# zafarrafii/REPET-Python

Hardware: AMD Instinct MI355X
Metric: audio-seconds/sec (x real-time) for repet.sim, 44.1 kHz stereo (higher is better)
Workload: dtype f32 (similarity GEMM: f16x3 split of the fp32 unit rows, fp32 accumulate; median: exact selection on bit-sliced rank codes)

## Files before the change

### repet-python_amd/csrc/peaks_exact.hip

```cpp
#include "peaks.h"
#include "fft_wave_f64.h"

#include <algorithm>
#include <cstdlib>
#include <type_traits>

namespace repet {

namespace {

#ifdef REPET_EXACT_STAMPS
#define XSTAMP_DECL unsigned long long xlast_ = wall_clock64();
#define XSTAMP(k) { __syncthreads(); if (threadIdx.x == 0) { const unsigned long long now_ = wall_clock64(); atomicAdd(&stats[24 + (k)], (unsigned)(now_ - xlast_)); xlast_ = now_; } }
#else
#define XSTAMP_DECL
#define XSTAMP(k)
#endif

#ifdef REPET_EXACT_STAMPS
__device__ unsigned long long g_unit_stamps[8];
#define USTAMP(k) { const unsigned long long now_ = wall_clock64(); if (lane == 0) atomicAdd(&g_unit_stamps[k], now_ - ulast_); ulast_ = now_; }
#define USTAMP_DECL unsigned long long ulast_ = wall_clock64();
#else
#define USTAMP(k)
#define USTAMP_DECL
#endif
constexpr int kExactThreads = 256, kExactWaves = kExactThreads / 64;
constexpr int kScanChunk = 4096;
constexpr int kRankLds = 512;
constexpr unsigned int kNear = 1, kSure = 2, kNeed1 = 4, kNeed2 = 8, kBand = 128;

struct ExactArgs {
    PeakArgs a;
    double delta2;
    const int* redo_list;
    ExactSource src;
    unsigned gen;
    int logM;
    unsigned char* scratch; size_t scratch_per_wg; int n4;
    int tw_count, fft_waves, wave_bytes, scan_in_lds;
    int reg_fft;
};

struct RowScratch {
    float* v; double* val; unsigned long long* best; unsigned int* st; int* list; int* list2; int* near; float* pval; int* pidx; int* prank;
};

__host__ __device__ inline size_t exact_row_scratch_bytes(int n4) {
    return (size_t)n4 * (8 + 8 + 4 + 4 + 4 + 4 + 4 + 4 + 4 + 4) + 256;
}

__device__ __forceinline__ RowScratch carve_row(unsigned char* p, int n4) {
    RowScratch r;
    r.val = reinterpret_cast<double*>(p); p += (size_t)n4 * 8;
    r.best = reinterpret_cast<unsigned long long*>(p); p += (size_t)n4 * 8;
    r.v = reinterpret_cast<float*>(p); p += (size_t)n4 * 4;
    r.list = reinterpret_cast<int*>(p); p += (size_t)n4 * 4;
    r.near = reinterpret_cast<int*>(p); p += (size_t)n4 * 4;
    r.pval = reinterpret_cast<float*>(p); p += (size_t)n4 * 4;
    r.pidx = reinterpret_cast<int*>(p); p += (size_t)n4 * 4;
    r.prank = reinterpret_cast<int*>(p); p += (size_t)n4 * 4;
    r.list2 = reinterpret_cast<int*>(p); p += (size_t)n4 * 4;
    r.st = reinterpret_cast<unsigned int*>(p);
    return r;
}

__device__ __forceinline__ void exact_wave_sync() {
    __builtin_amdgcn_fence(__ATOMIC_RELEASE, "wavefront");
    __builtin_amdgcn_wave_barrier();
    __builtin_amdgcn_fence(__ATOMIC_ACQUIRE, "wavefront");
}

template <bool ACC_REGS, bool STOCKHAM>
__device__ __forceinline__ void wave_unit_row_f64(const ExactSource& s, int logM, int clip, int64_t fr, double2* Zw, double* accw, const double2* tws, int lane) {
    const int W = s.W, M = W >> 1, F = s.F, C = s.n_channels;
    const int64_t s0 = s.frame_sample0 + fr * (int64_t)s.H;
    const float* hi = s.hi + (int64_t)clip * s.clip_stride;
    const float* lo = s.lo ? s.lo + (int64_t)clip * s.clip_stride : nullptr;
    const float* lo_or_hi = lo ? lo : hi;
    const double lo_scale = lo ? 1.0 : 0.0;
    int rel_lo = (int)min(max(-s0, (int64_t)0), (int64_t)W);
    int rel_hi = (int)min(max(s.n_samples - s0, (int64_t)0), (int64_t)W);
    const bool none = rel_hi <= rel_lo;
    const int64_t anchor = none ? 0 : s0;
    if (none) rel_hi = rel_lo + 1;
    const float* frame_hi = hi + anchor * C;
    const float* frame_lo = lo_or_hi + anchor * C;
    constexpr int kAcc = ACC_REGS ? 17 : 1;
    double acc[kAcc];
#pragma unroll
    for (int jj = 0; jj < kAcc; ++jj) acc[jj] = 0.0;
    if (!ACC_REGS) for (int k = lane; k <= M; k += 64) accw[k] = 0.0;
    for (int c = 0; c < C; ++c) {
        exact_wave_sync();
        for (int r0 = 0; r0 < M; r0 += 512) {
            float h0[8], h1[8], l0[8], l1[8];
            double w0[8], w1[8];
#pragma unroll
            for (int u = 0; u < 8; ++u) {
                const int r = min(r0 + 64 * u + lane, M - 1);
                const int q0 = min(max(2 * r, rel_lo), rel_hi - 1), q1 = min(max(2 * r + 1, rel_lo), rel_hi - 1);
                h0[u] = frame_hi[q0 * C + c]; h1[u] = frame_hi[q1 * C + c];
                l0[u] = frame_lo[q0 * C + c]; l1[u] = frame_lo[q1 * C + c];
                w0[u] = s.window64[2 * r]; w1[u] = s.window64[2 * r + 1];
            }
#pragma unroll
            for (int u = 0; u < 8; ++u) {
                const int r = r0 + 64 * u + lane;
                const int p0 = 2 * r;
                const bool in0 = !none && p0 >= rel_lo && p0 < rel_hi, in1 = !none && p0 + 1 >= rel_lo && p0 + 1 < rel_hi;
                const double re = in0 ? ((double)h0[u] + lo_scale * (double)l0[u]) * w0[u] : 0.0;
                const double im = in1 ? ((double)h1[u] + lo_scale * (double)l1[u]) * w1[u] : 0.0;
                if (r < M) Zw[STOCKHAM ? r : (int)(__brev((unsigned)r) >> (32 - logM))] = make_double2(re, im);
            }
        }
        exact_wave_sync();
        if constexpr (STOCKHAM) {
            for (int p = 1; p < M;) {
                if (M / p >= 4) {
                    const int tstep = M / (p * 4);
                    double2 u[4][4];
#pragma unroll
                    for (int b = 0; b < 4; ++b) {
                        const int i = min(lane + 64 * b, (M >> 2) - 1);
                        u[b][0] = Zw[i]; u[b][1] = Zw[i + (M >> 2)]; u[b][2] = Zw[i + (M >> 1)]; u[b][3] = Zw[i + 3 * (M >> 2)];
                    }
                    exact_wave_sync();
#pragma unroll
                    for (int b = 0; b < 4; ++b) {
                        const int i = lane + 64 * b;
                        if (i < (M >> 2)) {
                            const int k = i & (p - 1);
                            const int j = ((i - k) << 2) + k;
                            double2 u0 = u[b][0], u1 = u[b][1], u2 = u[b][2], u3 = u[b][3];
                            if (p > 1) {
                                const double2 w1 = tws[k * tstep], w2 = tws[2 * k * tstep], w3 = tws[3 * k * tstep];
                                u1 = make_double2(u1.x * w1.x - u1.y * w1.y, u1.x * w1.y + u1.y * w1.x);
                                u2 = make_double2(u2.x * w2.x - u2.y * w2.y, u2.x * w2.y + u2.y * w2.x);
                                u3 = make_double2(u3.x * w3.x - u3.y * w3.y, u3.x * w3.y + u3.y * w3.x);
                            }
                            const double2 t0 = make_double2(u0.x + u2.x, u0.y + u2.y), t1 = make_double2(u0.x - u2.x, u0.y - u2.y);
                            const double2 t2 = make_double2(u1.x + u3.x, u1.y + u3.y), d = make_double2(u1.x - u3.x, u1.y - u3.y);
                            const double2 t3 = make_double2(d.y, -d.x);
                            Zw[j] = make_double2(t0.x + t2.x, t0.y + t2.y);
                            Zw[j + p] = make_double2(t1.x + t3.x, t1.y + t3.y);
                            Zw[j + 2 * p] = make_double2(t0.x - t2.x, t0.y - t2.y);
                            Zw[j + 3 * p] = make_double2(t1.x - t3.x, t1.y - t3.y);
                        }
                    }
                    p *= 4;
                } else {
                    const int tstep = M / (p * 2);
                    double2 u[8][2];
#pragma unroll
                    for (int b = 0; b < 8; ++b) {
                        const int i = min(lane + 64 * b, (M >> 1) - 1);
                        u[b][0] = Zw[i]; u[b][1] = Zw[i + (M >> 1)];
                    }
                    exact_wave_sync();
#pragma unroll
                    for (int b = 0; b < 8; ++b) {
                        const int i = lane + 64 * b;
                        if (i < (M >> 1)) {
                            const int k = i & (p - 1);
                            const int j = ((i - k) << 1) + k;
                            const double2 w1 = tws[k * tstep];
                            const double2 u1 = make_double2(u[b][1].x * w1.x - u[b][1].y * w1.y, u[b][1].x * w1.y + u[b][1].y * w1.x);
                            Zw[j] = make_double2(u[b][0].x + u1.x, u[b][0].y + u1.y);
                            Zw[j + p] = make_double2(u[b][0].x - u1.x, u[b][0].y - u1.y);
                        }
                    }
                    p *= 2;
                }
                exact_wave_sync();
            }
        } else {
        for (int h = 1; h < M; h <<= 1) {
                const int ts = M / (2 * h);
                for (int b = lane; b < (M >> 1); b += 64) {
                    const int k = b & (h - 1);
                    const int i0 = ((b - k) << 1) + k, i1 = i0 + h;
                    const double2 w = tws ? tws[k * ts] : s.twiddle64[2 * k * ts];
                    const double2 u = Zw[i0], t = Zw[i1];
                    const double tr = t.x * w.x - t.y * w.y, ti = t.x * w.y + t.y * w.x;
                    Zw[i0] = make_double2(u.x + tr, u.y + ti);
                    Zw[i1] = make_double2(u.x - tr, u.y - ti);
                }
                exact_wave_sync();
            }
        }
        auto magnitude = [&](int k, double2 w) -> double {
            const double2 a = Zw[k & (M - 1)], b = Zw[(M - k) & (M - 1)];
            const double er = 0.5 * (a.x + b.x), ei = 0.5 * (a.y - b.y);
            const double dr = 0.5 * (a.x - b.x), di = 0.5 * (a.y + b.y);
            const double orr = di, oi = -dr;
            const double xr = er + orr * w.x - oi * w.y, xi = ei + orr * w.y + oi * w.x;
            return sqrt(xr * xr + xi * xi);
        };
        if (ACC_REGS) {
            double2 w[kAcc];
#pragma unroll
            for (int jj = 0; jj < kAcc; ++jj) w[jj] = s.twiddle64[min(lane + 64 * jj, M)];
#pragma unroll
            for (int jj = 0; jj < kAcc; ++jj) { const int k = min(lane + 64 * jj, M); const double m = magnitude(k, w[jj]); acc[jj] += (lane + 64 * jj <= M) ? m : 0.0; }
        } else {
            for (int k0 = 0; k0 <= M; k0 += 512) {
                double2 w[8];
#pragma unroll
                for (int u = 0; u < 8; ++u) w[u] = s.twiddle64[min(k0 + 64 * u + lane, M)];
#pragma unroll
                for (int u = 0; u < 8; ++u) { const int k = k0 + 64 * u + lane; if (k <= M) accw[k] += magnitude(k, w[u]); }
            }
        }
    }
    double part = 0.0;
    if (ACC_REGS) {
#pragma unroll
        for (int jj = 0; jj < kAcc; ++jj) { const int k = lane + 64 * jj; acc[jj] = acc[jj] / (double)C; if (k < F) part += acc[jj] * acc[jj]; }
    } else {
        exact_wave_sync();
        for (int k = lane; k < F; k += 64) { const double m = accw[k] / (double)C; accw[k] = m; part += m * m; }
        exact_wave_sync();
    }
    const double nrm = sqrt(wave_sum_f64(part));
    const bool mute = s.silent_zero && nrm == 0.0;
    double* out = s.u64 + (int64_t)clip * s.u64_clip_stride + fr * (int64_t)s.FS;
    if (ACC_REGS) {
#pragma unroll
        for (int jj = 0; jj < kAcc; ++jj) { const int k = lane + 64 * jj; if (k < s.FS) out[k] = (k < F && !mute) ? acc[jj] / nrm : 0.0; }
    } else {
        for (int k = lane; k < s.FS; k += 64) out[k] = (k < F && !mute) ? accw[k] / nrm : 0.0;
    }
}

__device__ __forceinline__ void wave_unit_row_f64_reg(const ExactSource& s, int clip, int64_t fr, double2* ex, const f64fft::Twiddles& tw, int lane) {
    constexpr int M = f64fft::kRegN;
    const int F = s.F, C = s.n_channels;
    const int64_t s0 = s.frame_sample0 + fr * (int64_t)s.H;
    const float* hi = s.hi + (int64_t)clip * s.clip_stride;
    const float* lo = s.lo ? s.lo + (int64_t)clip * s.clip_stride : nullptr;
    const float* lo_or_hi = lo ? lo : hi;
    const double lo_scale = lo ? 1.0 : 0.0;
    const int W2 = 2 * M;
    int rel_lo = (int)min(max(-s0, (int64_t)0), (int64_t)W2);
    int rel_hi = (int)min(max(s.n_samples - s0, (int64_t)0), (int64_t)W2);
    const bool none = rel_hi <= rel_lo;
    const int64_t anchor = none ? 0 : s0;
    if (none) rel_hi = rel_lo + 1;
    const float* frame_hi = hi + anchor * C;
    const float* frame_lo = lo_or_hi + anchor * C;
    double acc[17];
#pragma unroll
    for (int jj = 0; jj < 17; ++jj) acc[jj] = 0.0;
    USTAMP_DECL
    for (int c = 0; c < C; ++c) {
        double2 v[16];
        const bool pair_ok = !none && rel_lo == 0 && rel_hi == W2;
        if (pair_ok && C == 2) {
            struct __attribute__((packed, aligned(4))) F4 { float x, y, z, w; };
#pragma unroll
            for (int half = 0; half < 2; ++half) {
                float4 h4[8], l4[8];
                double2 w[8];
#pragma unroll
                for (int u = 0; u < 8; ++u) {
                    const int r = 64 * (8 * half + u) + lane;
                    const F4 a4 = *reinterpret_cast<const F4*>(frame_hi + 4 * r), b4 = *reinterpret_cast<const F4*>(frame_lo + 4 * r);
                    h4[u] = make_float4(a4.x, a4.y, a4.z, a4.w); l4[u] = make_float4(b4.x, b4.y, b4.z, b4.w);
                    w[u] = *reinterpret_cast<const double2*>(s.window64 + 2 * r);
                }
#pragma unroll
                for (int u = 0; u < 8; ++u) {
                    const float a0 = c ? h4[u].y : h4[u].x, a1 = c ? h4[u].w : h4[u].z, b0 = c ? l4[u].y : l4[u].x, b1 = c ? l4[u].w : l4[u].z;
                    v[8 * half + u] = make_double2(((double)a0 + lo_scale * (double)b0) * w[u].x, ((double)a1 + lo_scale * (double)b1) * w[u].y);
                }
                __builtin_amdgcn_sched_barrier(0);
            }
        } else if (pair_ok && C == 1) {
            struct __attribute__((packed, aligned(4))) F2 { float x, y; };
#pragma unroll
            for (int u = 0; u < 16; ++u) {
                const int r = 64 * u + lane;
                const F2 a2 = *reinterpret_cast<const F2*>(frame_hi + 2 * r), b2 = *reinterpret_cast<const F2*>(frame_lo + 2 * r);
                const double2 w = *reinterpret_cast<const double2*>(s.window64 + 2 * r);
                v[u] = make_double2(((double)a2.x + lo_scale * (double)b2.x) * w.x, ((double)a2.y + lo_scale * (double)b2.y) * w.y);
            }
            __builtin_amdgcn_sched_barrier(0);
        } else {
#pragma unroll
        for (int half = 0; half < 2; ++half) {
            float h0[8], h1[8], l0[8], l1[8];
            double2 w[8];
#pragma unroll
            for (int u = 0; u < 8; ++u) {
                const int r = 64 * (8 * half + u) + lane;
                const int q0 = min(max(2 * r, rel_lo), rel_hi - 1), q1 = min(max(2 * r + 1, rel_lo), rel_hi - 1);
                h0[u] = frame_hi[q0 * C + c]; h1[u] = frame_hi[q1 * C + c];
                l0[u] = frame_lo[q0 * C + c]; l1[u] = frame_lo[q1 * C + c];
                w[u] = *reinterpret_cast<const double2*>(s.window64 + 2 * r);
            }
#pragma unroll
            for (int u = 0; u < 8; ++u) {
                const int p0 = 2 * (64 * (8 * half + u) + lane);
                const bool in0 = !none && p0 >= rel_lo && p0 < rel_hi, in1 = !none && p0 + 1 >= rel_lo && p0 + 1 < rel_hi;
                v[8 * half + u] = make_double2(in0 ? ((double)h0[u] + lo_scale * (double)l0[u]) * w[u].x : 0.0,
                                               in1 ? ((double)h1[u] + lo_scale * (double)l1[u]) * w[u].y : 0.0);
            }
            __builtin_amdgcn_sched_barrier(0);
        }
        }
        USTAMP(0)
        f64fft::wave_fft1024(v, ex, tw, lane);
        __builtin_amdgcn_sched_barrier(0);
        USTAMP(1)
#pragma unroll
        for (int sl = 0; sl < 16; ++sl) ex[lane + 64 * sl] = v[sl];
        f64fft::wave_fence();
#pragma unroll
        for (int j0 = 0; j0 < 18; j0 += 6) {
            double2 tw_k[6];
#pragma unroll
            for (int u = 0; u < 6; ++u) tw_k[u] = s.twiddle64[min(lane + 64 * (j0 + u), M)];
#pragma unroll
            for (int u = 0; u < 6; ++u) {
                const int jj = j0 + u;
                if (jj < 17) {
                    const int k = min(lane + 64 * jj, M);
                    const double2 a = ex[k & (M - 1)], b = ex[(M - k) & (M - 1)];
                    const double er = 0.5 * (a.x + b.x), ei = 0.5 * (a.y - b.y);
                    const double dr = 0.5 * (a.x - b.x), di = 0.5 * (a.y + b.y);
                    const double orr = di, oi = -dr;
                    const double xr = er + orr * tw_k[u].x - oi * tw_k[u].y, xi = ei + orr * tw_k[u].y + oi * tw_k[u].x;
                    const double m = sqrt(xr * xr + xi * xi);
                    acc[jj] += (lane + 64 * jj <= M) ? m : 0.0;
                }
            }
            __builtin_amdgcn_sched_barrier(0);
        }
        f64fft::wave_fence();
        USTAMP(2)
    }
    double part = 0.0;
#pragma unroll
    for (int jj = 0; jj < 17; ++jj) { const int k = lane + 64 * jj; acc[jj] = acc[jj] / (double)C; if (k < F) part += acc[jj] * acc[jj]; }
    const double nrm = sqrt(wave_sum_f64(part));
    const bool mute = s.silent_zero && nrm == 0.0;
    double* out = s.u64 + (int64_t)clip * s.u64_clip_stride + fr * (int64_t)s.FS;
#pragma unroll
    for (int jj = 0; jj < 17; ++jj) { const int k = lane + 64 * jj; if (k < s.FS) out[k] = (k < F && !mute) ? acc[jj] / nrm : 0.0; }
    USTAMP(3)
}

constexpr int kFftReg = 0, kFftLds4 = 1, kFftLdsAcc = 2;
template <int V>
__device__ __forceinline__ void unit_row_variant(const ExactSource& src, int logM, int clip, int64_t fr, double2* Zw, double* accw,
                                                 const double2* tws, const f64fft::Twiddles& rtw, int lane) {
    if constexpr (V == kFftReg) wave_unit_row_f64_reg(src, clip, fr, Zw, rtw, lane);
    else if constexpr (V == kFftLds4) wave_unit_row_f64<false, true>(src, logM, clip, fr, Zw, accw, tws, lane);
    else wave_unit_row_f64<false, false>(src, logM, clip, fr, Zw, accw, tws, lane);
}

struct FftPlan { int variant, tw_count, wave_bytes, fixed_bytes; };
static FftPlan fft_plan(int W, bool allow_reg = true) {
    const int Mh = W / 2;
    FftPlan p{};
    if (W == 2048 && allow_reg) {
        p.variant = kFftReg; p.tw_count = 0; p.wave_bytes = f64fft::kExPitch * (int)sizeof(double2);
        p.fixed_bytes = f64fft::kTwCount * (int)sizeof(double2);
    } else if (W <= 2048) {
        p.variant = kFftLds4; p.tw_count = Mh;
        p.wave_bytes = Mh * (int)sizeof(double2) + (Mh + 8) * (int)sizeof(double);
        p.fixed_bytes = p.tw_count * (int)sizeof(double2);
    } else {
        p.variant = kFftLdsAcc; p.tw_count = Mh / 2;
        p.wave_bytes = Mh * (int)sizeof(double2) + (Mh + 8) * (int)sizeof(double);
        p.fixed_bytes = p.tw_count * (int)sizeof(double2);
        if (p.fixed_bytes + p.wave_bytes > 150 * 1024) { p.tw_count = 0; p.fixed_bytes = 0; }
    }
    return p;
}

struct UnitRowsArgs {
    ExactSource src; const int* frame_list; unsigned int* stats; unsigned int gen;
    int logM;
};

template <int KQ>
__global__ __launch_bounds__(256, KQ == 1 ? 4 : 1) void unit_rows_f64_wg_kernel(UnitRowsArgs x) {
    constexpr int kWgQ = KQ;
    constexpr int kCP = KQ == 1 ? 2 : 1;
    extern __shared__ __attribute__((aligned(16))) unsigned char wg_smem[];
    const ExactSource& s = x.src;
    const int tid = threadIdx.x, lane = tid & 63, wave = tid >> 6;
    const int W = s.W, M = W >> 1, F = s.F, C = s.n_channels;
    if (x.stats[11] >= x.stats[10]) return;
    constexpr bool kHalfTw = KQ == 1;
    const int n_tw = kHalfTw ? M >> 1 : M;
    double2* tw_lds = reinterpret_cast<double2*>(wg_smem);
    double2* Z = tw_lds + n_tw;
    double* red = reinterpret_cast<double*>(Z);
    for (int k = tid; k < n_tw; k += 256) tw_lds[k] = s.twiddle64[2 * k];
    auto tw = [&](int m) -> double2 {
        if constexpr (!kHalfTw) return tw_lds[m];
        else {
            const double2 v = tw_lds[m & ((M >> 1) - 1)];
            return (m & (M >> 1)) ? make_double2(-v.x, -v.y) : v;
        }
    };
    const unsigned int n_frames = x.stats[10];
    const int nq = (M + 255) >> 8;
    for (unsigned int slot = blockIdx.x; slot < n_frames; slot += gridDim.x) {
        __syncthreads();
        const int64_t lin = x.frame_list[slot];
        if (s.u64_gen[lin] == x.gen) continue;
        const int clip = (int)(lin / s.gen_clip_stride);
        const int64_t fr = lin - (int64_t)clip * s.gen_clip_stride;
        unsigned int* g = s.u64_gen + lin;
        const int64_t s0 = s.frame_sample0 + fr * (int64_t)s.H;
        const float* hi = s.hi + (int64_t)clip * s.clip_stride;
        const float* lo = s.lo ? s.lo + (int64_t)clip * s.clip_stride : hi;
        const double lo_scale = s.lo ? 1.0 : 0.0;
        int rel_lo = (int)min(max(-s0, (int64_t)0), (int64_t)W);
        int rel_hi = (int)min(max(s.n_samples - s0, (int64_t)0), (int64_t)W);
        const bool none = rel_hi <= rel_lo;
        if (none) { rel_lo = 0; rel_hi = 1; }
        const float* frame_hi = hi + (none ? 0 : s0) * C;
        const float* frame_lo = lo + (none ? 0 : s0) * C;
        const bool whole = !none && rel_lo == 0 && rel_hi == W;
        double acc[kWgQ * 4 + 1];
#pragma unroll
        for (int q = 0; q < kWgQ * 4 + 1; ++q) acc[q] = 0.0;
        for (int c0 = 0; c0 < C; c0 += kCP) {
            const int nc = min(kCP, C - c0);
            for (int q0 = 0; q0 < nq; q0 += 4) {
                float h0[kCP][4], h1[kCP][4], l0[kCP][4], l1[kCP][4];
                double2 w[4];
#pragma unroll
                for (int u = 0; u < 4; ++u) {
                    const int r = min(tid + 256 * (q0 + u), M - 1);
                    const int a0 = min(max(2 * r, rel_lo), rel_hi - 1), a1 = min(max(2 * r + 1, rel_lo), rel_hi - 1);
#pragma unroll
                    for (int cc = 0; cc < kCP; ++cc) {
                        const int c = min(c0 + cc, C - 1);
                        h0[cc][u] = frame_hi[a0 * C + c]; h1[cc][u] = frame_hi[a1 * C + c];
                        l0[cc][u] = frame_lo[a0 * C + c]; l1[cc][u] = frame_lo[a1 * C + c];
                    }
                    w[u] = *reinterpret_cast<const double2*>(s.window64 + 2 * r);
                }
#pragma unroll
                for (int u = 0; u < 4; ++u) {
                    const int r = tid + 256 * (q0 + u);
                    const int p0 = 2 * r;
                    const bool in0 = !none && (whole || (p0 >= rel_lo && p0 < rel_hi)), in1 = !none && (whole || (p0 + 1 >= rel_lo && p0 + 1 < rel_hi));
#pragma unroll
                    for (int cc = 0; cc < kCP; ++cc)
                        if (r < M && cc < nc) Z[cc * M + r] = make_double2(in0 ? ((double)h0[cc][u] + lo_scale * (double)l0[cc][u]) * w[u].x : 0.0,
                                                                          in1 ? ((double)h1[cc][u] + lo_scale * (double)l1[cc][u]) * w[u].y : 0.0);
                }
            }
            __syncthreads();
            for (int p = 1; p < M;) {
                if (M / p >= 4) {
                    const int tstep = M / (p * 4), quarter = M >> 2;
                    double2 u[kCP][kWgQ][4];
#pragma unroll
                    for (int cc = 0; cc < kCP; ++cc)
#pragma unroll
                        for (int b = 0; b < kWgQ; ++b) {
                            const int i = min(tid + 256 * b, quarter - 1);
                            const double2* Zc = Z + (cc < nc ? cc : 0) * M;
                            u[cc][b][0] = Zc[i]; u[cc][b][1] = Zc[i + quarter]; u[cc][b][2] = Zc[i + 2 * quarter]; u[cc][b][3] = Zc[i + 3 * quarter];
                        }
                    __syncthreads();
#pragma unroll
                    for (int cc = 0; cc < kCP; ++cc)
#pragma unroll
                        for (int b = 0; b < kWgQ; ++b) {
                            const int i = tid + 256 * b;
                            if (i < quarter && cc < nc) {
                                double2* Zc = Z + cc * M;
                                const int k = i & (p - 1);
                                const int j = ((i - k) << 2) + k;
                                double2 u0 = u[cc][b][0], u1 = u[cc][b][1], u2 = u[cc][b][2], u3 = u[cc][b][3];
                                if (p > 1) {
                                    const double2 w1 = tw(k * tstep), w2 = tw(2 * k * tstep), w3 = tw(3 * k * tstep);
                                    u1 = make_double2(u1.x * w1.x - u1.y * w1.y, u1.x * w1.y + u1.y * w1.x);
                                    u2 = make_double2(u2.x * w2.x - u2.y * w2.y, u2.x * w2.y + u2.y * w2.x);
                                    u3 = make_double2(u3.x * w3.x - u3.y * w3.y, u3.x * w3.y + u3.y * w3.x);
                                }
                                const double2 t0 = make_double2(u0.x + u2.x, u0.y + u2.y), t1 = make_double2(u0.x - u2.x, u0.y - u2.y);
                                const double2 t2 = make_double2(u1.x + u3.x, u1.y + u3.y), d = make_double2(u1.x - u3.x, u1.y - u3.y);
                                const double2 t3 = make_double2(d.y, -d.x);
                                Zc[j] = make_double2(t0.x + t2.x, t0.y + t2.y);
                                Zc[j + p] = make_double2(t1.x + t3.x, t1.y + t3.y);
                                Zc[j + 2 * p] = make_double2(t0.x - t2.x, t0.y - t2.y);
                                Zc[j + 3 * p] = make_double2(t1.x - t3.x, t1.y - t3.y);
                            }
                        }
                    p *= 4;
                } else {
                    const int tstep = M / (p * 2), half = M >> 1;
                    double2 u[kCP][2 * kWgQ][2];
#pragma unroll
                    for (int cc = 0; cc < kCP; ++cc)
#pragma unroll
                        for (int b = 0; b < 2 * kWgQ; ++b) {
                            const int i = min(tid + 256 * b, half - 1);
                            const double2* Zc = Z + (cc < nc ? cc : 0) * M;
                            u[cc][b][0] = Zc[i]; u[cc][b][1] = Zc[i + half];
                        }
                    __syncthreads();
#pragma unroll
                    for (int cc = 0; cc < kCP; ++cc)
#pragma unroll
                        for (int b = 0; b < 2 * kWgQ; ++b) {
                            const int i = tid + 256 * b;
                            if (i < half && cc < nc) {
                                double2* Zc = Z + cc * M;
                                const int k = i & (p - 1);
                                const int j = ((i - k) << 1) + k;
                                const double2 w1 = tw(k * tstep);
                                const double2 u1 = make_double2(u[cc][b][1].x * w1.x - u[cc][b][1].y * w1.y, u[cc][b][1].x * w1.y + u[cc][b][1].y * w1.x);
                                Zc[j] = make_double2(u[cc][b][0].x + u1.x, u[cc][b][0].y + u1.y);
                                Zc[j + p] = make_double2(u[cc][b][0].x - u1.x, u[cc][b][0].y - u1.y);
                            }
                        }
                    p *= 2;
                }
                __syncthreads();
            }
#pragma unroll
            for (int q = 0; q < kWgQ * 4 + 1; ++q) {
                const int kk = tid + 256 * q;
                if (q <= nq) {
                    const int k = min(kk, M);
                    const double2 wk = s.twiddle64[k];
#pragma unroll
                    for (int cc = 0; cc < kCP; ++cc) {
                        if (cc >= nc) break;
                        const double2* Zc = Z + cc * M;
                        const double2 a = Zc[k & (M - 1)], b = Zc[(M - k) & (M - 1)];
                        const double er = 0.5 * (a.x + b.x), ei = 0.5 * (a.y - b.y);
                        const double dr = 0.5 * (a.x - b.x), di = 0.5 * (a.y + b.y);
                        const double orr = di, oi = -dr;
                        const double xr = er + orr * wk.x - oi * wk.y, xi = ei + orr * wk.y + oi * wk.x;
                        const double m = sqrt(xr * xr + xi * xi);
                        acc[q] += (kk <= M) ? m : 0.0;
                    }
                }
            }
            __syncthreads();
        }
        double part = 0.0;
#pragma unroll
        for (int q = 0; q < kWgQ * 4 + 1; ++q) {
            const int k = tid + 256 * q;
            acc[q] = acc[q] / (double)C;
            if (k < F) part += acc[q] * acc[q];
        }
        part = wave_sum_f64(part);
        if (lane == 0) red[wave] = part;
        __syncthreads();
        const double nrm = sqrt(red[0] + red[1] + red[2] + red[3]);
        const bool mute = s.silent_zero && nrm == 0.0;
        double* out = s.u64 + (int64_t)clip * s.u64_clip_stride + fr * (int64_t)s.FS;
#pragma unroll
        for (int q = 0; q < kWgQ * 4 + 1; ++q) {
            const int k = tid + 256 * q;
            if (k < s.FS) out[k] = (k < F && !mute) ? acc[q] / nrm : 0.0;
        }
        if (tid == 0) { *g = x.gen; stat_add(x.stats, 9, 1u); }
    }
}

template <int V>
__global__ __launch_bounds__(kExactThreads) void local_maxima_exact_kernel(ExactArgs x) {
    extern __shared__ __attribute__((aligned(16))) unsigned char exact_smem[];
    __shared__ int sh_slot, n_near, n_list, n_list2, n_peak, n_band, n_above;
    __shared__ float cutv[2];
    __shared__ double red[kExactWaves], red2[kExactWaves];
    __shared__ float s_pval[kRankLds];
    __shared__ int s_pidx[kRankLds];
    const int tid = threadIdx.x, lane = tid & 63, wave = tid >> 6;
    const int M = x.src.W >> 1;
    RowScratch R = carve_row(x.scratch + (size_t)blockIdx.x * x.scratch_per_wg, x.n4);
    unsigned int* stats = x.a.stats;
    if (stats[5] >= stats[4]) return;
    const double2* tws = nullptr;
    unsigned char* work = exact_smem;
    f64fft::Twiddles rtw{nullptr, nullptr};
    if (x.reg_fft) {
        rtw = f64fft::load_twiddles(reinterpret_cast<double2*>(exact_smem), x.src.twiddle64, tid, kExactThreads);
        work += (size_t)f64fft::kTwCount * sizeof(double2);
    } else if (x.tw_count > 0) {
        double2* t = reinterpret_cast<double2*>(exact_smem);
        for (int k = tid; k < x.tw_count; k += kExactThreads) t[k] = x.src.twiddle64[2 * k];
        tws = t;
        work += (size_t)x.tw_count * sizeof(double2);
    }

    for (;;) {
        __syncthreads();
        if (tid == 0) sh_slot = (int)atomicAdd(&stats[5], 1u);
        __syncthreads();
        const int slot = sh_slot;
        if (slot >= (int)stats[4]) return;
        PeakArgs a = x.a;
        const int64_t r = x.redo_list[2 * slot];
        const int clip = x.redo_list[2 * slot + 1];
        a.M += clip * a.m_stride;
        a.idx += clip * a.idx_stride;
        a.count += clip * a.cnt_stride;
        a.unit += clip * a.unit_stride;
        apply_origin(a, clip);
        const int d = a.d;
        const int64_t j = a.row0 + r;
        const int n = row_columns(a, j);
        const float dlt = a.delta;
        const double d2 = x.delta2, thr64 = a.min_value64;
        auto lag_of = [&](int i) -> int { int l = (int)(j - i) % n; return l < 0 ? l + n : l; };
        auto fetch = [&](int i) -> float {
            if (a.mode == 0) return a.M[j * a.pitch + i];
            const int l = lag_of(i);
            return a.M[(a.mode == 2 ? j - a.shift : j - l - a.shift) * a.pitch + l];
        };
        auto frame_of = [&](int i) -> int64_t { return a.mode == 0 ? (int64_t)i : j - lag_of(i) - a.shift; };
        auto out_index = [&](int i) -> int { return a.mode == 0 ? i : (int)(j - lag_of(i) - a.shift); };
        const int64_t self_fr = j - a.shift;
        const float* self32 = a.unit + self_fr * (int64_t)a.unit_pitch;
        const int len4 = a.unit_pitch >> 2;

        XSTAMP_DECL
        if (tid == 0) { n_near = 0; n_list = 0; n_list2 = 0; n_peak = 0; n_band = 0; n_above = 0; }
        __syncthreads();
        for (int i0 = 0; i0 < x.n4; i0 += 8 * kExactThreads) {
            float e[8];
#pragma unroll
            for (int u = 0; u < 8; ++u) e[u] = fetch(min(i0 + kExactThreads * u + tid, n - 1));
#pragma unroll
            for (int u = 0; u < 8; ++u) {
                const int i = i0 + kExactThreads * u + tid;
                if (i < x.n4) { R.v[i] = i < n ? (a.silent_zero ? peak_value<true>(e[u]) : nan_to_inf(e[u])) : -INFINITY; R.st[i] = 0u; }
            }
        }
        __syncthreads();
        auto candidate = [&](int i, float vi, float mx) {
            if (vi < mx - dlt) return;
            const bool sure = (vi >= a.min_value + dlt) && (vi > mx + dlt);
            if (sure) { R.st[i] = kSure; const int p = atomicAdd(&n_peak, 1); R.pidx[p] = i; R.pval[p] = vi; }
            else { R.st[i] = kNear | kNeed1; R.near[atomicAdd(&n_near, 1)] = i; R.list[atomicAdd(&n_list, 1)] = i; }
        };
        if (x.scan_in_lds) {
            int w = 1;
            while (2 * w <= d) w *= 2;
            const int blen = kScanChunk + 2 * d + 8;
            float* bufA = reinterpret_cast<float*>(work);
            float* bufB = bufA + blen;
            for (int c0 = 0; c0 < n; c0 += kScanChunk) {
                const int lo = c0 - d, t_hi = c0 + kScanChunk < n ? c0 + kScanChunk : n, len = t_hi + d - lo;
                __syncthreads();
                for (int e0 = 0; e0 < len; e0 += 8 * kExactThreads) {
                    float t8[8];
#pragma unroll
                    for (int u = 0; u < 8; ++u) t8[u] = R.v[min(max(lo + e0 + kExactThreads * u + tid, 0), n - 1)];
#pragma unroll
                    for (int u = 0; u < 8; ++u) {
                        const int e = e0 + kExactThreads * u + tid, i = lo + e;
                        if (e < len) bufA[e] = (i >= 0 && i < n) ? t8[u] : -INFINITY;
                    }
                }
                __syncthreads();
                float* src = bufA;
                float* dst = bufB;
                for (int step = 1; step < w; step *= 2) {
                    for (int e = tid; e < len; e += kExactThreads) dst[e] = fmaxf(src[e], e + step < len ? src[e + step] : -INFINITY);
                    __syncthreads();
                    float* t = src; src = dst; dst = t;
                }
                for (int i = c0 + tid; i < t_hi; i += kExactThreads) {
                    const float vi = R.v[i];
                    if (!(vi < INFINITY) || vi < a.min_value - dlt) continue;
                    float mx = -INFINITY;
                    if (d > 0) {
                        const int e = i - lo;
                        mx = fmaxf(fmaxf(src[e - d], src[e - w]), fmaxf(src[e + 1], src[e + d - w + 1]));
                    }
                    candidate(i, vi, mx);
                }
            }
        } else {
            for (int i = tid; i < n; i += kExactThreads) {
                const float vi = R.v[i];
                if (!(vi < INFINITY) || vi < a.min_value - dlt) continue;
                const int k_lo = i - d > 0 ? i - d : 0, k_hi = i + d < n - 1 ? i + d : n - 1;
                float mx = -INFINITY;
                for (int k = k_lo; k <= k_hi; ++k) {
                    if (k != i) mx = fmaxf(mx, R.v[k]);
                    if (mx > vi + dlt) break;
                }
                candidate(i, vi, mx);
            }
        }
        __syncthreads();
        const int nn = n_near;
        const int win = 2 * d + 1;
        const long long n_pairs = (long long)nn * win;
        auto for_rival_pairs = [&](auto&& fn) {
            for (long long e = tid; e < n_pairs; e += kExactThreads) {
                const int q = (int)(e / win);
                const int i = R.near[q];
                const int k = i - d + (int)(e - (long long)q * win);
                if (k == i || k < 0 || k >= n) continue;
                if (!(R.v[k] >= R.v[i] - dlt)) continue;
                fn(q, i, k);
            }
        };
        for_rival_pairs([&](int, int, int k) { if (!(atomicOr(&R.st[k], kNeed1) & kNeed1)) R.list[atomicAdd(&n_list, 1)] = k; });
        __syncthreads();

        int list_done = 0;
        auto level1 = [&]() {
            __syncthreads();
            const int items = n_list;
            for (int it = list_done + 2 * wave; it < items; it += 2 * kExactWaves) {
                const bool two = it + 1 < items;
                const int i0 = R.list[it], i1 = R.list[two ? it + 1 : it];
                double e0, e1;
                exact_similarity2(self32, a.unit + frame_of(i0) * (int64_t)a.unit_pitch, a.unit + frame_of(i1) * (int64_t)a.unit_pitch,
                                  len4, lane, &e0, &e1);
                if (lane == 0) { R.val[i0] = e0; if (two) R.val[i1] = e1; }
            }
            list_done = items;
            __syncthreads();
        };
        int list2_done = 0;
        auto level2 = [&]() {
            __syncthreads();
            const int first = list2_done, items = n_list2 - list2_done;
            list2_done = n_list2;
            if (items == 0) return;
            unsigned* gens = x.src.u64_gen + (int64_t)clip * x.src.gen_clip_stride;
            if (wave < x.fft_waves) {
                double2* Zw = reinterpret_cast<double2*>(work + (size_t)wave * x.wave_bytes);
                double* accw = reinterpret_cast<double*>(Zw + M);
                for (int it = wave - 1; it < items; it += x.fft_waves) {
                    const int64_t fr = it < 0 ? self_fr : frame_of(R.list2[first + it]);
                    if (__hip_atomic_load(&gens[fr], __ATOMIC_ACQUIRE, __HIP_MEMORY_SCOPE_AGENT) == x.gen) continue;
                    unit_row_variant<V>(x.src, x.logM, clip, fr, Zw, accw, tws, rtw, lane);
                    __threadfence();
                    if (lane == 0) {
                        __hip_atomic_store(&gens[fr], x.gen, __ATOMIC_RELEASE, __HIP_MEMORY_SCOPE_AGENT);
                        stat_add(stats, 9, 1u);
                    }
                }
            }
            __threadfence();
            __syncthreads();
            const double* base = x.src.u64 + (int64_t)clip * x.src.u64_clip_stride;
            const double* self64 = base + self_fr * (int64_t)x.src.FS;
            double worst = 0.0;
            for (int it = wave; it < items; it += kExactWaves) {
                const int i = R.list2[first + it];
                const double e = dot_rows_f64(self64, base + frame_of(i) * (int64_t)x.src.FS, x.src.FS, lane);
                if (lane == 0) {
                    const double diff = fabs(e - R.val[i]);
                    if (diff > worst) worst = diff;
                    R.val[i] = e;
                }
            }
            if (lane == 0 && worst > 0.0) stat_max(stats, 8, (unsigned)fmin(worst * 1e12, 4.0e9));
            if (tid == 0) stat_add(stats, 6, (unsigned)items);
            __syncthreads();
        };
        auto best_rivals = [&]() {
            for (int q = tid; q < nn; q += kExactThreads) R.best[q] = 0ull;
            __syncthreads();
            for_rival_pairs([&](int q, int, int k) { atomicMax(&R.best[q], (unsigned long long)__double_as_longlong(R.val[k]) + 1ull); });
            __syncthreads();
        };

        XSTAMP(0)
        level1();
        XSTAMP(1)
        best_rivals();
        for (int q = tid; q < nn; q += kExactThreads) {
            const int i = R.near[q];
            const double ei = R.val[i];
            const unsigned long long b = R.best[q];
            const bool versus_rival = b != 0ull && fabs(ei - __longlong_as_double((long long)(b - 1ull))) < d2;
            R.prank[q] = versus_rival ? 1 : 0;
            if (versus_rival || fabs(ei - thr64) < d2) { if (!(atomicOr(&R.st[i], kNeed2) & kNeed2)) R.list2[atomicAdd(&n_list2, 1)] = i; }
        }
        __syncthreads();
        for_rival_pairs([&](int q, int, int k) {
            if (R.prank[q] && R.val[k] > __longlong_as_double((long long)(R.best[q] - 1ull)) - d2) { if (!(atomicOr(&R.st[k], kNeed2) & kNeed2)) R.list2[atomicAdd(&n_list2, 1)] = k; }
        });
        XSTAMP(2)
        level2();
        XSTAMP(3)
        best_rivals();
        for (int q = tid; q < nn; q += kExactThreads) {
            const int i = R.near[q];
            const double ei = R.val[i];
            const unsigned long long b = R.best[q];
            if (ei >= thr64 && (b == 0ull || ei > __longlong_as_double((long long)(b - 1ull)))) {
                const int p = atomicAdd(&n_peak, 1);
                R.pidx[p] = i;
                R.pval[p] = (float)ei;
            }
        }
        __syncthreads();

        XSTAMP(4)
        const int np_ = n_peak;
        const int kept = np_ < a.number ? np_ : a.number;
        int* out = a.idx + r * (int64_t)a.idx_pitch;
        int differs = 0;
        const int old_count = a.count[r];
        const float* pv = R.pval;
        const int* pi = R.pidx;
        if (np_ <= kRankLds) {
            for (int p = tid; p < np_; p += kExactThreads) { s_pval[p] = R.pval[p]; s_pidx[p] = R.pidx[p]; }
            __syncthreads();
            pv = s_pval; pi = s_pidx;
        }
        for (int p = tid; p < np_; p += kExactThreads) {
            const float v = pv[p];
            const int i = pi[p];
            int rank = 0;
            for (int q = 0; q < np_; ++q) {
                const float u = pv[q];
                rank += (u > v) || (u == v && pi[q] > i);
            }
            R.prank[p] = rank;
        }
        __syncthreads();
        if (np_ > a.number) {
            for (int p = tid; p < np_; p += kExactThreads) {
                if (R.prank[p] == a.number - 1) cutv[0] = R.pval[p];
                if (R.prank[p] == a.number) cutv[1] = R.pval[p];
            }
            __syncthreads();
            const float c_in = cutv[0], c_out = cutv[1];
            if (c_in - c_out <= dlt) {
                const float lo = c_out - dlt, hi = c_in + dlt;
                for (int p = tid; p < np_; p += kExactThreads) {
                    const float v = R.pval[p];
                    if (v > hi) atomicAdd(&n_above, 1);
                    else if (v >= lo) { R.near[atomicAdd(&n_band, 1)] = p; const int i = R.pidx[p]; if (!(atomicOr(&R.st[i], kNeed1 | kBand) & kNeed1)) R.list[atomicAdd(&n_list, 1)] = i; }
                }
                level1();
                const int nb = n_band;
                const int above = n_above;
                auto rank_band = [&]() {
                    for (int q = tid; q < nb; q += kExactThreads) {
                        const int p = R.near[q];
                        const int i = R.pidx[p];
                        const double e = R.val[i];
                        int crank = 0;
                        for (int t = 0; t < nb; ++t) {
                            const int k = R.pidx[R.near[t]];
                            const double ek = R.val[k];
                            crank += (ek > e) || (ek == e && k > i);
                        }
                        R.prank[p] = above + crank;
                    }
                    __syncthreads();
                };
                rank_band();
                double low_kept = INFINITY, high_dropped = -INFINITY;
                for (int q = tid; q < nb; q += kExactThreads) {
                    const int p = R.near[q];
                    const double e = R.val[R.pidx[p]];
                    if (R.prank[p] < a.number) low_kept = fmin(low_kept, e); else high_dropped = fmax(high_dropped, e);
                }
                for (int sh = 32; sh > 0; sh >>= 1) {
                    low_kept = fmin(low_kept, __shfl_xor(low_kept, sh));
                    high_dropped = fmax(high_dropped, __shfl_xor(high_dropped, sh));
                }
                __syncthreads();
                if (lane == 0) { red[wave] = low_kept; red2[wave] = high_dropped; }
                __syncthreads();
                for (int k = 0; k < kExactWaves; ++k) { low_kept = fmin(low_kept, red[k]); high_dropped = fmax(high_dropped, red2[k]); }
                if (low_kept - high_dropped < d2) {
                    for (int q = tid; q < nb; q += kExactThreads) {
                        const int p = R.near[q];
                        const int i = R.pidx[p];
                        const double e = R.val[i];
                        const bool kept_now = R.prank[p] < a.number;
                        if ((kept_now && e < high_dropped + d2) || (!kept_now && e > low_kept - d2)) { if (!(atomicOr(&R.st[i], kNeed2) & kNeed2)) R.list2[atomicAdd(&n_list2, 1)] = i; }
                    }
                    level2();
                    rank_band();
                }
                __syncthreads();
            }
        }
        for (int p = tid; p < np_; p += kExactThreads) {
            const int rank = R.prank[p];
            if (rank < a.number) {
                const int o = out_index(R.pidx[p]);
                if (rank >= old_count || out[rank] != o) differs = 1;
                out[rank] = o;
            }
        }
        for (int k = kept + tid; k < a.number; k += kExactThreads) out[k] = -1;
        if (kept != old_count) differs = 1;
        const int any = __syncthreads_or(differs);
        if (tid == 0) {
            a.count[r] = kept;
            if (any) stat_add(stats, 7, 1u);
        }
        XSTAMP(5)
    }
}

}

#ifdef REPET_EXACT_STAMPS
extern "C" int repet_debug_unit_stamps(unsigned long long* out) {
    const int rc = (int)hipMemcpyFromSymbol(out, HIP_SYMBOL(g_unit_stamps), sizeof(unsigned long long) * 8);
    unsigned long long zero[8] = {};
    (void)hipMemcpyToSymbol(HIP_SYMBOL(g_unit_stamps), zero, sizeof(zero));
    return rc;
}
#endif

size_t local_maxima_exact_scratch_bytes(int32_t n_cols, int* grid_out) {
    const int n4 = (int)round_up(n_cols, 4) + 4;
    const size_t per = round_up((int64_t)exact_row_scratch_bytes(n4), 256);
    int64_t grid = 512;
    const int64_t budget = (int64_t)2 << 30;
    if ((int64_t)per * grid > budget) grid = std::max<int64_t>(64, budget / (int64_t)per);
    if (grid_out) *grid_out = (int)grid;
    return per * (size_t)grid;
}

hipError_t launch_local_maxima_exact(const float* M, int64_t row0, int32_t n_cols, int64_t pitch, int32_t mode, float min_value,
                                     int32_t d, int32_t number, int32_t* idx, int32_t idx_pitch, int32_t* count, hipStream_t s,
                                     int64_t shift, const PeakRefine* refine, const PeakBatch* batch, const ExactSource& src,
                                     void* scratch, PeakLaunch* info) {
    if (!refine || !refine->unit_rows || !(refine->delta > 0.0f) || !refine->redo_list || !refine->stats) return hipSuccess;
    if (d > n_cols) d = n_cols;
    ExactArgs x{};
    PeakArgs& a = x.a;
    a.M = M; a.row0 = row0; a.n = n_cols; a.pitch = pitch; a.mode = mode; a.min_value = min_value; a.d = d;
    a.number = number; a.idx = idx; a.idx_pitch = idx_pitch; a.count = count; a.shift = shift;
    a.unit = refine->unit_rows; a.unit_pitch = refine->pitch; a.delta = refine->delta;
    a.min_value64 = refine->min_value; a.stats = refine->stats;
    a.start = (batch && batch->start > 0) ? batch->start : n_cols;
    a.silent_zero = (refine->silent_zero && mode != 0) ? 1 : 0;
    if (batch && batch->n_batch > 0) {
        a.m_stride = batch->m_stride; a.idx_stride = batch->idx_stride; a.cnt_stride = batch->cnt_stride;
        a.unit_stride = batch->unit_stride;
        if (mode != 0) a.origin = batch->origin;
    }
    x.delta2 = refine->delta2; x.redo_list = refine->redo_list; x.src = src; x.gen = refine->gen;
    int logM = 0;
    while ((2 << logM) < src.W) ++logM;
    x.logM = logM;
    int grid = 0;
    const size_t total = local_maxima_exact_scratch_bytes(n_cols, &grid);
    x.n4 = (int)round_up(n_cols, 4) + 4;
    x.scratch = static_cast<unsigned char*>(scratch);
    x.scratch_per_wg = total / grid;
    const FftPlan plan = fft_plan(src.W, false);
    x.reg_fft = 0; x.tw_count = plan.tw_count; x.wave_bytes = plan.wave_bytes;
    const int small = 76 * 1024, large = 150 * 1024;
    const int fixed = plan.fixed_bytes;
    int waves = 4;
    while (waves > 1 && fixed + waves * x.wave_bytes > small) --waves;
    if (waves < 2) { waves = 4; while (waves > 1 && fixed + waves * x.wave_bytes > large) --waves; }
    x.fft_waves = waves;
    int work = waves * x.wave_bytes;
    const int scan_bytes = 2 * (kScanChunk + 2 * d + 8) * (int)sizeof(float);
    if (fixed + scan_bytes <= std::max(fixed + work, small)) { x.scan_in_lds = 1; work = std::max(work, scan_bytes); }
    const int lds = fixed + work;
    auto go = [&](auto tag) -> hipError_t {
        constexpr int V = decltype(tag)::value;
        hipError_t e = ensure_dynamic_lds(reinterpret_cast<const void*>(&local_maxima_exact_kernel<V>), lds);
        if (e != hipSuccess) return e;
        hipLaunchKernelGGL(local_maxima_exact_kernel<V>, dim3((unsigned)grid), dim3(kExactThreads), lds, s, x);
        return hipGetLastError();
    };
    if (info) info->exact_fft = plan.variant == kFftLds4 ? kFftLds4 : kFftLdsAcc;
    if (plan.variant == kFftLds4) return go(std::integral_constant<int, kFftLds4>{});
    return go(std::integral_constant<int, kFftLdsAcc>{});
}

hipError_t launch_unit_rows_f64(const ExactSource& src, const PeakRefine* refine, hipStream_t s, PeakLaunch* info) {
    if (!refine || !refine->frame_list || !refine->stats) return hipSuccess;
    UnitRowsArgs x{};
    x.src = src; x.frame_list = refine->frame_list; x.stats = refine->stats; x.gen = refine->gen;
    int logM = 0;
    while ((2 << logM) < src.W) ++logM;
    x.logM = logM;
    const int Mh = src.W / 2;
    const int lds = Mh <= 1024 ? (Mh / 2 + 2 * Mh) * (int)sizeof(double2) : 2 * Mh * (int)sizeof(double2);
    auto go_wg = [&](auto tag) -> hipError_t {
        constexpr int KQ = decltype(tag)::value;
        hipError_t e = ensure_dynamic_lds(reinterpret_cast<const void*>(&unit_rows_f64_wg_kernel<KQ>), lds);
        if (e != hipSuccess) return e;
        hipLaunchKernelGGL(unit_rows_f64_wg_kernel<KQ>, dim3(1024), dim3(256), lds, s, x);
        return hipGetLastError();
    };
    if (info) info->unit_kq = Mh <= 1024 ? 1 : 4;
    return Mh <= 1024 ? go_wg(std::integral_constant<int, 1>{}) : go_wg(std::integral_constant<int, 4>{});
}

}
```

Measured before the change: 218,600.

## Specialise small-window unit-row kernel to 512 threads with per-channel-pair parallel FFT

Adds a 512-thread specialisation of the fp64 unit-row kernel for windows up to 2048, where each 256-thread half of the workgroup runs the FFT of one channel of a stereo pair at the same time instead of processing channels sequentially. Magnitudes are accumulated directly into registers and then normalised through an LDS bin buffer. The generic template is now restricted to the larger-window case. The aim is to cut per-frame latency of the exact unit-row refinement and raise occupancy, at the cost of more LDS per block and more code.

```diff
diff --git a/repet-python_amd/csrc/peaks_exact.hip b/repet-python_amd/csrc/peaks_exact.hip
--- a/repet-python_amd/csrc/peaks_exact.hip
+++ b/repet-python_amd/csrc/peaks_exact.hip
@@ -385,28 +385,23 @@
     int logM;
 };
 
+constexpr int kUnitThreads = 512;
 template <int KQ>
-__global__ __launch_bounds__(256, KQ == 1 ? 4 : 1) void unit_rows_f64_wg_kernel(UnitRowsArgs x) {
+__global__ __launch_bounds__(256, 1) void unit_rows_f64_wg_kernel(UnitRowsArgs x) {
+    static_assert(KQ > 1, "windows up to 2048 take the 512-thread specialisation");
     constexpr int kWgQ = KQ;
-    constexpr int kCP = KQ == 1 ? 2 : 1;
+    constexpr int kCP = 1;
     extern __shared__ __attribute__((aligned(16))) unsigned char wg_smem[];
     const ExactSource& s = x.src;
     const int tid = threadIdx.x, lane = tid & 63, wave = tid >> 6;
     const int W = s.W, M = W >> 1, F = s.F, C = s.n_channels;
     if (x.stats[11] >= x.stats[10]) return;
-    constexpr bool kHalfTw = KQ == 1;
-    const int n_tw = kHalfTw ? M >> 1 : M;
+    const int n_tw = M;
     double2* tw_lds = reinterpret_cast<double2*>(wg_smem);
     double2* Z = tw_lds + n_tw;
     double* red = reinterpret_cast<double*>(Z);
     for (int k = tid; k < n_tw; k += 256) tw_lds[k] = s.twiddle64[2 * k];
-    auto tw = [&](int m) -> double2 {
-        if constexpr (!kHalfTw) return tw_lds[m];
-        else {
-            const double2 v = tw_lds[m & ((M >> 1) - 1)];
-            return (m & (M >> 1)) ? make_double2(-v.x, -v.y) : v;
-        }
-    };
+    auto tw = [&](int m) -> double2 { return tw_lds[m]; };
     const unsigned int n_frames = x.stats[10];
     const int nq = (M + 255) >> 8;
     for (unsigned int slot = blockIdx.x; slot < n_frames; slot += gridDim.x) {
@@ -570,6 +565,256 @@
             if (k < s.FS) out[k] = (k < F && !mute) ? acc[q] / nrm : 0.0;
         }
         if (tid == 0) { *g = x.gen; stat_add(x.stats, 9, 1u); }
+    }
+}
+
+template <>
+__global__ __launch_bounds__(kUnitThreads, 8) void unit_rows_f64_wg_kernel<1>(UnitRowsArgs x) {
+    extern __shared__ __attribute__((aligned(16))) unsigned char wg_smem[];
+    const ExactSource& s = x.src;
+    const int tid = threadIdx.x;
+    const int W = s.W, M = W >> 1, F = s.F, C = s.n_channels;
+    USTAMP_DECL
+#ifdef REPET_EXACT_STAMPS
+    const unsigned long long born_ = ulast_;
+#endif
+    if (x.stats[11] >= x.stats[10]) return;
+    const int n_tw = M >> 1;
+    double2* tw_lds = reinterpret_cast<double2*>(wg_smem);
+    double2* Z = tw_lds + n_tw;
+    double* red = reinterpret_cast<double*>(Z);
+    double* bins = red + 8;
+    for (int k = tid; k < n_tw; k += kUnitThreads) tw_lds[k] = s.twiddle64[2 * k];
+    auto tw = [&](int m) -> double2 {
+        const double2 v = tw_lds[m & ((M >> 1) - 1)];
+        return (m & (M >> 1)) ? make_double2(-v.x, -v.y) : v;
+    };
+    const unsigned int n_frames = x.stats[10];
+    for (unsigned int slot = blockIdx.x; slot < n_frames; slot += gridDim.x) {
+        __syncthreads();
+        const int64_t lin = x.frame_list[slot];
+        if (s.u64_gen[lin] == x.gen) continue;
+        int tv = tid;
+        asm volatile("" : "+v"(tv));
+        const int lane = tv & 63, wave = tv >> 6;
+        const int cc = tv >> 8, t = tv & 255;
+        USTAMP(0)
+        const int clip = (int)(lin / s.gen_clip_stride);
+        const int64_t fr = lin - (int64_t)clip * s.gen_clip_stride;
+        unsigned int* g = s.u64_gen + lin;
+        const int64_t s0 = s.frame_sample0 + fr * (int64_t)s.H;
+        const float* hi = s.hi + (int64_t)clip * s.clip_stride;
+        const float* lo = s.lo ? s.lo + (int64_t)clip * s.clip_stride : hi;
+        const double lo_scale = s.lo ? 1.0 : 0.0;
+        int rel_lo = (int)min(max(-s0, (int64_t)0), (int64_t)W);
+        int rel_hi = (int)min(max(s.n_samples - s0, (int64_t)0), (int64_t)W);
+        const bool none = rel_hi <= rel_lo;
+        if (none) { rel_lo = 0; rel_hi = 1; }
+        const float* frame_hi = hi + (none ? 0 : s0) * C;
+        const float* frame_lo = lo + (none ? 0 : s0) * C;
+        const bool whole = !none && rel_lo == 0 && rel_hi == W;
+        double* out = s.u64 + (int64_t)clip * s.u64_clip_stride + fr * (int64_t)s.FS;
+        double acc0, acc1, acc_m;
+        for (int c0 = 0; c0 < C; c0 += 2) {
+            int tl = tid;
+            asm volatile("" : "+v"(tl));
+            const int nc = min(2, C - c0);
+            const double2 wsplit1 = s.twiddle64[min(2 * tl + 1, M)];
+            const double2 wsplit_m = s.twiddle64[M];
+            auto put = [&](int r, int ch, float a0, float a1, float b0, float b1, double2 w, bool in0, bool in1) {
+                if (r < M && ch < nc) Z[ch * M + r] = make_double2(in0 ? ((double)a0 + lo_scale * (double)b0) * w.x : 0.0,
+                                                                  in1 ? ((double)a1 + lo_scale * (double)b1) * w.y : 0.0);
+            };
+            for (int r0 = 0; r0 < M; r0 += 2 * kUnitThreads) {
+                double2 w[2];
+                if (whole && C == 2) {
+                    struct __attribute__((packed, aligned(4))) F4 { float x, y, z, w; };
+                    float4 h4[2], l4[2];
+#pragma unroll
+                    for (int u = 0; u < 2; ++u) {
+                        const int r = min(r0 + tl + kUnitThreads * u, M - 1);
+                        const F4 a4 = *reinterpret_cast<const F4*>(frame_hi + 4 * r);
+                        h4[u] = make_float4(a4.x, a4.y, a4.z, a4.w);
+                        w[u] = *reinterpret_cast<const double2*>(s.window64 + 2 * r);
+                    }
+#pragma unroll
+                    for (int u = 0; u < 2; ++u) {
+                        l4[u] = h4[u];
+                        if (s.lo) {
+                            const F4 b4 = *reinterpret_cast<const F4*>(frame_lo + 4 * min(r0 + tl + kUnitThreads * u, M - 1));
+                            l4[u] = make_float4(b4.x, b4.y, b4.z, b4.w);
+                        }
+                    }
+#pragma unroll
+                    for (int u = 0; u < 2; ++u) {
+                        const int r = r0 + tl + kUnitThreads * u;
+                        put(r, 0, h4[u].x, h4[u].z, l4[u].x, l4[u].z, w[u], true, true);
+                        put(r, 1, h4[u].y, h4[u].w, l4[u].y, l4[u].w, w[u], true, true);
+                    }
+                } else if (whole && C == 1) {
+                    struct __attribute__((packed, aligned(4))) F2 { float x, y; };
+                    float2 h2[2], l2[2];
+#pragma unroll
+                    for (int u = 0; u < 2; ++u) {
+                        const int r = min(r0 + tl + kUnitThreads * u, M - 1);
+                        const F2 a2 = *reinterpret_cast<const F2*>(frame_hi + 2 * r);
+                        h2[u] = make_float2(a2.x, a2.y);
+                        w[u] = *reinterpret_cast<const double2*>(s.window64 + 2 * r);
+                    }
+#pragma unroll
+                    for (int u = 0; u < 2; ++u) {
+                        l2[u] = h2[u];
+                        if (s.lo) {
+                            const F2 b2 = *reinterpret_cast<const F2*>(frame_lo + 2 * min(r0 + tl + kUnitThreads * u, M - 1));
+                            l2[u] = make_float2(b2.x, b2.y);
+                        }
+                    }
+#pragma unroll
+                    for (int u = 0; u < 2; ++u) put(r0 + tl + kUnitThreads * u, 0, h2[u].x, h2[u].y, l2[u].x, l2[u].y, w[u], true, true);
+                } else {
+                    float h0[2][2], h1[2][2], l0[2][2], l1[2][2];
+#pragma unroll
+                    for (int u = 0; u < 2; ++u) {
+                        const int r = min(r0 + tl + kUnitThreads * u, M - 1);
+                        const int a0 = min(max(2 * r, rel_lo), rel_hi - 1), a1 = min(max(2 * r + 1, rel_lo), rel_hi - 1);
+#pragma unroll
+                        for (int ch = 0; ch < 2; ++ch) {
+                            const int c = min(c0 + ch, C - 1);
+                            h0[ch][u] = frame_hi[a0 * C + c]; h1[ch][u] = frame_hi[a1 * C + c];
+                            l0[ch][u] = frame_lo[a0 * C + c]; l1[ch][u] = frame_lo[a1 * C + c];
+                        }
+                        w[u] = *reinterpret_cast<const double2*>(s.window64 + 2 * r);
+                    }
+#pragma unroll
+                    for (int u = 0; u < 2; ++u) {
+                        const int r = r0 + tl + kUnitThreads * u;
+                        const int p0 = 2 * r;
+                        const bool in0 = !none && p0 >= rel_lo && p0 < rel_hi, in1 = !none && p0 + 1 >= rel_lo && p0 + 1 < rel_hi;
+#pragma unroll
+                        for (int ch = 0; ch < 2; ++ch) put(r, ch, h0[ch][u], h1[ch][u], l0[ch][u], l1[ch][u], w[u], in0, in1);
+                    }
+                }
+            }
+            __syncthreads();
+            USTAMP(1)
+            const bool live = cc < nc;
+            double2* Zc = Z + (live ? cc : 0) * M;
+            for (int p = 1; p < M;) {
+                if (M / p >= 4) {
+                    const int tstep = M / (p * 4), quarter = M >> 2;
+                    const int il = min(t, quarter - 1);
+                    double2 u0 = Zc[il], u1 = Zc[il + quarter], u2 = Zc[il + 2 * quarter], u3 = Zc[il + 3 * quarter];
+                    __syncthreads();
+                    if (t < quarter && live) {
+                        const int i = t;
+                        const int k = i & (p - 1);
+                        const int j = ((i - k) << 2) + k;
+                        if (p > 1) {
+                            const double2 w1 = tw(k * tstep), w2 = tw(2 * k * tstep), w3 = tw(3 * k * tstep);
+                            u1 = make_double2(u1.x * w1.x - u1.y * w1.y, u1.x * w1.y + u1.y * w1.x);
+                            u2 = make_double2(u2.x * w2.x - u2.y * w2.y, u2.x * w2.y + u2.y * w2.x);
+                            u3 = make_double2(u3.x * w3.x - u3.y * w3.y, u3.x * w3.y + u3.y * w3.x);
+                        }
+                        const double2 t0 = make_double2(u0.x + u2.x, u0.y + u2.y), t1 = make_double2(u0.x - u2.x, u0.y - u2.y);
+                        const double2 t2 = make_double2(u1.x + u3.x, u1.y + u3.y), d = make_double2(u1.x - u3.x, u1.y - u3.y);
+                        const double2 t3 = make_double2(d.y, -d.x);
+                        Zc[j] = make_double2(t0.x + t2.x, t0.y + t2.y);
+                        Zc[j + p] = make_double2(t1.x + t3.x, t1.y + t3.y);
+                        Zc[j + 2 * p] = make_double2(t0.x - t2.x, t0.y - t2.y);
+                        Zc[j + 3 * p] = make_double2(t1.x - t3.x, t1.y - t3.y);
+                    }
+                    p *= 4;
+                } else {
+                    const int tstep = M / (p * 2), half = M >> 1;
+                    double2 u[2][2];
+#pragma unroll
+                    for (int b = 0; b < 2; ++b) {
+                        const int i = min(t + 256 * b, half - 1);
+                        u[b][0] = Zc[i]; u[b][1] = Zc[i + half];
+                    }
+                    __syncthreads();
+#pragma unroll
+                    for (int b = 0; b < 2; ++b) {
+                        const int i = t + 256 * b;
+                        if (i < half && live) {
+                            const int k = i & (p - 1);
+                            const int j = ((i - k) << 1) + k;
+                            const double2 w1 = tw(k * tstep);
+                            const double2 u1 = make_double2(u[b][1].x * w1.x - u[b][1].y * w1.y, u[b][1].x * w1.y + u[b][1].y * w1.x);
+                            Zc[j] = make_double2(u[b][0].x + u1.x, u[b][0].y + u1.y);
+                            Zc[j + p] = make_double2(u[b][0].x - u1.x, u[b][0].y - u1.y);
+                        }
+                    }
+                    p *= 2;
+                }
+                __syncthreads();
+            }
+            USTAMP(2)
+            int tq = tid;
+            asm volatile("" : "+v"(tq));
+            auto split_bin = [&](int k, double2 wk, double& acc) {
+#pragma unroll
+                for (int ch = 0; ch < 2; ++ch) {
+                    if (ch >= nc) break;
+                    const double2* Zh = Z + ch * M;
+                    const double2 a = Zh[k & (M - 1)], b = Zh[(M - k) & (M - 1)];
+                    const double er = 0.5 * (a.x + b.x), ei = 0.5 * (a.y - b.y);
+                    const double dr = 0.5 * (a.x - b.x), di = 0.5 * (a.y + b.y);
+                    const double orr = di, oi = -dr;
+                    const double xr = er + orr * wk.x - oi * wk.y, xi = ei + orr * wk.y + oi * wk.x;
+                    const double m = sqrt(xr * xr + xi * xi);
+                    acc += m;
+                }
+            };
+            const bool have = 2 * tq < M;
+            acc0 = 0.0; acc1 = 0.0; acc_m = 0.0;
+            if (c0 > 0) {
+                if (have) { acc0 = out[2 * tq]; acc1 = out[2 * tq + 1]; }
+                if (tid == 0) acc_m = out[M];
+            }
+            if (have) {
+                split_bin(2 * tq, tw_lds[min(tq, n_tw - 1)], acc0);
+                split_bin(2 * tq + 1, wsplit1, acc1);
+            }
+            if (tid == 0) split_bin(M, wsplit_m, acc_m);
+            if (c0 + 2 < C) {
+                if (have) { out[2 * tq] = acc0; out[2 * tq + 1] = acc1; }
+                if (tid == 0) out[M] = acc_m;
+            }
+            __syncthreads();
+            USTAMP(3)
+        }
+        int tb = tid;
+        asm volatile("" : "+v"(tb));
+        acc0 = acc0 / (double)C; acc1 = acc1 / (double)C; acc_m = acc_m / (double)C;
+        if (2 * tb < M) { bins[2 * tb] = acc0; bins[2 * tb + 1] = acc1; }
+        if (tid == 0) bins[M] = acc_m;
+        __syncthreads();
+        if (wave < 4) {
+            double part = 0.0;
+#pragma unroll
+            for (int q = 0; q < 5; ++q) {
+                const int k = t + 256 * q;
+                if (k < F && k <= M) { const double v = bins[k]; part += v * v; }
+            }
+            part = wave_sum_f64(part);
+            if (lane == 0) red[wave] = part;
+        }
+        __syncthreads();
+        const double nrm = sqrt(red[0] + red[1] + red[2] + red[3]);
+        USTAMP(4)
+        const bool mute = s.silent_zero && nrm == 0.0;
+        if (2 * tb < M) {
+            out[2 * tb] = (2 * tb < F && !mute) ? acc0 / nrm : 0.0;
+            out[2 * tb + 1] = (2 * tb + 1 < F && !mute) ? acc1 / nrm : 0.0;
+        }
+        for (int k = M + 1 + tb; k < s.FS; k += kUnitThreads) out[k] = 0.0;
+        if (tid == 0) out[M] = (M < F && !mute) ? acc_m / nrm : 0.0;
+        if (tid == 0) { *g = x.gen; stat_add(x.stats, 9, 1u); }
+        USTAMP(5)
+#ifdef REPET_EXACT_STAMPS
+        if (lane == 0) { atomicAdd(&g_unit_stamps[6], 1ull); atomicMax(&g_unit_stamps[7], ulast_ - born_); }
+#endif
     }
 }
 
@@ -1001,7 +1246,7 @@
         constexpr int KQ = decltype(tag)::value;
         hipError_t e = ensure_dynamic_lds(reinterpret_cast<const void*>(&unit_rows_f64_wg_kernel<KQ>), lds);
         if (e != hipSuccess) return e;
-        hipLaunchKernelGGL(unit_rows_f64_wg_kernel<KQ>, dim3(1024), dim3(256), lds, s, x);
+        hipLaunchKernelGGL(unit_rows_f64_wg_kernel<KQ>, dim3(1024), dim3(KQ == 1 ? kUnitThreads : 256), lds, s, x);
         return hipGetLastError();
     };
     if (info) info->unit_kq = Mh <= 1024 ? 1 : 4;
```

Result: no change. 219,300 (median of 5 runs) (+0.3%).
